# maua-maua-maua/maua

Measured on AMD Instinct MI355X. Metric: frames/sec (whole node), 1024x1024 StyleGAN2 audio-reactive render, higher is better.
Workload: dtype bf16

## Files before the change

maua_amd/csrc/common.h:

```cpp
#pragma once
#include <hip/hip_runtime.h>
#include <stdint.h>
#include <string>

#include "../../include/maua_hip.h"

namespace maua {

typedef __attribute__((ext_vector_type(8))) __bf16 bf16x8;
typedef __attribute__((ext_vector_type(16))) float f32x16;
typedef __attribute__((ext_vector_type(4))) float f32x4;
typedef __attribute__((ext_vector_type(4))) uint32_t u32x4;

typedef uint16_t bf16_t;

__device__ __forceinline__ float bf2f(bf16_t v) { return __uint_as_float(((uint32_t)v) << 16); }
typedef __bf16 hw_bf16x2 __attribute__((ext_vector_type(2)));
typedef float f32x2_t __attribute__((ext_vector_type(2)));
__device__ __forceinline__ uint32_t pack2bf(float lo, float hi) {
  const f32x2_t v = {lo, hi};
  return __builtin_bit_cast(uint32_t, __builtin_convertvector(v, hw_bf16x2));
}
__device__ __forceinline__ bf16_t f2bf(float f) { return (bf16_t)(pack2bf(f, 0.f) & 0xffffu); }

// ... 87 lines not shown

__device__ __forceinline__ void lds_dma_b128(const void* sbase, unsigned voff_bytes, void* lds_wave_base) {
  const unsigned base =
      __builtin_amdgcn_readfirstlane((unsigned)(size_t)(__attribute__((address_space(3))) void*)lds_wave_base);
  asm volatile("s_mov_b32 m0, %2\n\ts_nop 0\n\tglobal_load_lds_dwordx4 %0, %1" ::"v"(voff_bytes), "s"(sbase), "s"(base)
               : "memory");
}

void set_error(const std::string& msg);
int fail(const std::string& msg);
#define MAUA_HIP_CHECK(expr)                                                                  \
  do {                                                                                        \
    hipError_t _e = (expr);                                                                   \
    if (_e != hipSuccess)                                                                     \
      return ::maua::fail(std::string(#expr) + ": " + hipGetErrorString(_e));                 \
  } while (0)
#define MAUA_REQUIRE(cond, msg)                                   \
  do {                                                            \
    if (!(cond)) return ::maua::fail(std::string(msg));           \
  } while (0)

static inline int cdiv(int a, int b) { return (a + b - 1) / b; }

}

struct maua_ctx {
  int device;
  hipStream_t stream;
  void* scratch = nullptr;
  size_t scratch_bytes = 0;
  int dma_conv = 1;
  int gemm_dma = 1;
  int linear_dma = 0;
};

namespace maua {
int scratch_reserve(maua_ctx* ctx, size_t bytes);
}
```

maua_amd/csrc/context.hip:

```cpp
#include "common.h"

namespace maua {
static thread_local std::string g_err;
void set_error(const std::string& msg) { g_err = msg; }
int fail(const std::string& msg) {
  g_err = msg;
  return MAUA_ERR;
}
int scratch_reserve(maua_ctx* ctx, size_t bytes) {
  if (bytes <= ctx->scratch_bytes) return MAUA_OK;
  MAUA_HIP_CHECK(hipStreamSynchronize(ctx->stream));
  if (ctx->scratch) MAUA_HIP_CHECK(hipFree(ctx->scratch));
  ctx->scratch = nullptr;
  ctx->scratch_bytes = 0;
  size_t want = bytes + bytes / 4;
  MAUA_HIP_CHECK(hipMalloc(&ctx->scratch, want));
  ctx->scratch_bytes = want;
  return MAUA_OK;
}
}

namespace {
__global__ void clock_stamp_kernel(unsigned long long* stamp) {
  stamp[0] = __builtin_amdgcn_s_memtime();
// ... 9 lines not shown
int maua_ctx_create(int device, void* stream, maua_ctx** out) {
  MAUA_REQUIRE(out != nullptr, "maua_ctx_create: out is NULL");
  int n = 0;
  MAUA_HIP_CHECK(hipGetDeviceCount(&n));
  MAUA_REQUIRE(device >= 0 && device < n, "maua_ctx_create: no such HIP device (this library has no CPU fallback)");
  MAUA_HIP_CHECK(hipSetDevice(device));
  maua_ctx* c = new maua_ctx();
  c->device = device;
  c->stream = (hipStream_t)stream;
  *out = c;
  return MAUA_OK;
}

int maua_ctx_set_stream(maua_ctx* ctx, void* stream) {
  MAUA_REQUIRE(ctx != nullptr, "maua_ctx_set_stream: ctx is NULL");
  ctx->stream = (hipStream_t)stream;
  return MAUA_OK;
}

int maua_ctx_set_option(maua_ctx* ctx, const char* key, int value) {
  MAUA_REQUIRE(ctx && key, "maua_ctx_set_option: NULL argument");
  if (std::string(key) == "dma_conv") {
    ctx->dma_conv = value;
    return MAUA_OK;
  }
  if (std::string(key) == "linear_dma") {
    ctx->linear_dma = value;
    return MAUA_OK;
  }
  if (std::string(key) == "gemm_dma") {
    ctx->gemm_dma = value;
    return MAUA_OK;
  }
  return maua::fail(std::string("maua_ctx_set_option: unknown option ") + key);
}

int maua_ctx_sync(maua_ctx* ctx) {
  MAUA_REQUIRE(ctx != nullptr, "maua_ctx_sync: ctx is NULL");
  MAUA_HIP_CHECK(hipStreamSynchronize(ctx->stream));
  return MAUA_OK;
}

int maua_ctx_clock_stamp(maua_ctx* ctx, unsigned long long* stamp_dev) {
  MAUA_REQUIRE(ctx && stamp_dev, "maua_ctx_clock_stamp: NULL argument");
  hipLaunchKernelGGL(clock_stamp_kernel, dim3(1), dim3(1), 0, ctx->stream, stamp_dev);
  MAUA_HIP_CHECK(hipGetLastError());
  return MAUA_OK;
}

void maua_ctx_destroy(maua_ctx* ctx) {
  if (!ctx) return;
  if (ctx->scratch) {
    hipStreamSynchronize(ctx->stream);
    hipFree(ctx->scratch);
  }
  delete ctx;
}

}
```

maua_amd/csrc/internal.h:

```cpp
#pragma once
#include "common.h"

namespace maua {

int launch_pack_rgb8(hipStream_t stream, const float* img, uint8_t* out, int B, int H, int W);
template <typename TI, typename TO>
int launch_nchw_to_nhwc(hipStream_t s, const void* x, void* y, int N, int C, int HW, int Cp);
template <typename TI, typename TO>
int launch_nhwc_to_nchw(hipStream_t s, const void* x, void* y, int N, int C, int HW, int Cp);

struct ConvArgs {
  const void* x;
  long x_bstride;
  const void* w;
  const float* s;
  const float* d;
  const float* noise;
  long noise_bstride;
  float noise_strength;
  const float* noise_scale;
  const float* bias;
  void* y;
  int B, H, W, Ci, Co, up;
  int act;
// ... 61 lines not shown
  long noise_bstride;
  float noise_strength;
  const float* noise_scale;
  const float* bias;
  void* y;
  int B, H, W, Ci, Co, up, act;
  float alpha, gain, clamp;
  const float* rgb_wmod;
  const float* rgb_bias;
  const float* rgb_prev;
  float* rgb_out;
  float rgb_clamp;
  float fir[16];
  uint8_t* rgb8_out;
  int rgb_skip_f32;
};
bool hires_supported(int dtype, int Ci, int Co, int up, int H, int W);
int launch_modconv_hires(hipStream_t stream, const HiresArgs& a, int dtype = MAUA_BF16);
bool upwalk_supported(int dtype, int Ci, int Co, int up, int H, int W);
size_t upwalk_weight_elems(int Co, int Ci);
int launch_upwalk(hipStream_t stream, const HiresArgs& a, int dtype = MAUA_BF16);
int launch_prep_upwalk_weights(hipStream_t stream, const float* w, void* wt, int Co, int Ci, int flip, int dtype = MAUA_BF16);
bool upwalk_fused_supported(int dtype, int Ci, int Cm, int H, int W);
int launch_upwalk_fused(hipStream_t stream, const HiresArgs& up, const HiresArgs& c1, int force_segs = 0, int narrow_ok = 1,
                        int dtype = MAUA_BF16);

int launch_prep_weights(hipStream_t stream, int dtype, const float* w, void* wt, float* wsq, int Co, int Ci, int k,
                        int up, int flip, int Cop, int Cip);
int launch_f32_split_inplace(hipStream_t stream, void* w, long n_floats);

int launch_tconv2(hipStream_t stream, int dtype, const ConvArgs& a);
bool tconv_dma_supported(int dtype, int Ci, int Co, int H, int W);
int launch_tconv_dma(hipStream_t stream, const ConvArgs& a, int dtype = MAUA_BF16);
int launch_tconv_edges(hipStream_t stream, const ConvArgs& a, int dtype = MAUA_BF16);
int launch_prep_tconv_weights(hipStream_t stream, int dtype, const float* w, void* wt, int Co, int Ci, int flip);

struct UpfirArgs {
  const void* t;
  void* y;
  const float* d;
  const float* noise;
  long noise_bstride;
  float noise_strength;
  const float* noise_scale;
  const float* bias;
  const float* out_scale;
  int B, H, W, Co;
  int act;
  float alpha, gain, clamp;
};
int launch_upfir_epilogue(hipStream_t stream, int dtype, const UpfirArgs& a);
bool tconv_fir_supported(int dtype, int Ci, int Co, int H, int W);
int launch_tconv_fir(hipStream_t stream, const ConvArgs& a, const UpfirArgs& u, int dtype = MAUA_BF16, int walk = 1, int force_segs = 0);
size_t prepped_weight_elems(int k, int up, int Cop, int Cip);

struct LayerOperands { const void* x; const void* w; const float* s; const float* d; const float* bias; void* y; int B, H, W, Ci, Co, up; };
struct NoiseOperands { const float* noise; long bstride; float strength; const float* scale; };
struct Epilogue { int act; float alpha, gain, clamp; };
template <typename A>
inline void set_noise_args(A& a, const NoiseOperands& n) {
  a.noise = n.noise; a.noise_bstride = n.bstride; a.noise_strength = n.strength; a.noise_scale = n.scale;
}
template <typename A>
inline void set_epilogue_args(A& a, const Epilogue& e) {
  a.act = e.act; a.alpha = e.alpha; a.gain = e.gain; a.clamp = e.clamp;
}
template <typename A>
// ... 60 lines not shown
int launch_resize2d(hipStream_t stream, int dtype, bool nhwc, const ResizeArgs& a);
int launch_skip_add(hipStream_t stream, const float* y, const float* prev, float* out, int B, int H, int W,
                    const float* fir16);
int launch_warp_affine_nhwc(hipStream_t stream, int dtype, const void* x, void* y, const float* minv, int B, int H, int W,
                            int C);

struct StyleLayer {
  const float* affine_w;
  const float* affine_b;
  const float* wsq;
  const float* wrgb;
  float* s;
  float* d;
  float* wmod;
  int w_index;
  int Cin, Co, Cs, Cd;
  float scale;
};
int launch_styles(hipStream_t stream, const StyleLayer* layers_dev, int n_layers, const float* ws, int num_ws,
                  int w_dim, int B, int max_channels, int f16_prenorm = 0);
int launch_f16_prenorm_weights(hipStream_t stream, const float* w, float* out, int Co, int Ci, int kk);
int launch_f16_prenorm_styles(hipStream_t stream, float* s, int B, int Cs, int Cin);

struct RgbArgs {
  const void* x;
  const float* wmod;
  const float* bias;
  const float* prev;
  float* out;
  int B, H, W, C;
  float clamp;
  float fir[16];
};
int launch_torgb(hipStream_t stream, int dtype, const RgbArgs& a);

struct GemmArgs {
  const void* a0; long lda0; int K0;
  const void* a1; long lda1; int K1;
  const void* w;
  const float* bias;
  const void* res;
  long ldr;
  void* c;
  long ldc;
  long M;
  int N;
  int c_f32;
  int prefer_dma;
  int epi;
  void* c2; long ldc2;
  const void* aux; long ldaux;
  int batch;
  long a_bstride, w_bstride, c_bstride;
  int remap_nt;
};
int launch_gemm_nt(hipStream_t stream, int dtype, const GemmArgs& g);
struct GemmRoute { int kernel; int remap_nt; };
GemmRoute gemm_route(int dtype, const GemmArgs& g, int prefer_dma, int force = 0);
int gemm_plan(int dtype, const GemmArgs& g, int prefer_dma, int force, GemmRoute* out);
int launch_gemm_routed(hipStream_t stream, int dtype, const GemmArgs& g, GemmRoute r);
bool gemm_dma_shape_ok(int dtype, const GemmArgs& g);
bool gemm_dma_supported(int dtype, const GemmArgs& g);
bool gemm256_shape_ok(const GemmArgs& g);
bool gemm256_takes(const GemmArgs& g);
int launch_gemm_dma(hipStream_t stream, const GemmArgs& g, int kernel);

struct AttnArgs {
// ... 125 lines not shown
```

maua_amd/csrc/modconv.hip:

```cpp
#include <cstdlib>

#include "common.h"
#include "internal.h"

namespace maua {


template <typename T> struct Mma;
template <> struct Mma<bf16_t> {
  using FW = u32x4;
  using FX = u32x4;
  __device__ static __forceinline__ FW prep_w(const u32x4& v) { return v; }
  __device__ static __forceinline__ FX prep_x(const u32x4& v) { return v; }
  __device__ static __forceinline__ void step(f32x16& acc, const u32x4& a, const u32x4& b) {
    acc = __builtin_amdgcn_mfma_f32_32x32x16_bf16(__builtin_bit_cast(bf16x8, a), __builtin_bit_cast(bf16x8, b), acc, 0,
                                                  0, 0);
  }
  __device__ static __forceinline__ u32x4 scale(const u32x4& v, const float* sv) {
    u32x4 o;
#pragma unroll
    for (int k = 0; k < 4; k++)
      o[k] = pack2bf(bf2f((bf16_t)(v[k] & 0xffff)) * sv[2 * k], bf2f((bf16_t)(v[k] >> 16)) * sv[2 * k + 1]);
    return o;
  }
// ... 872 lines not shown
      if constexpr (sizeof(T) == 2) {
        xv[0] = Fmt16<T>::lo(v.x); xv[1] = Fmt16<T>::hi(v.x);
        xv[2] = Fmt16<T>::lo(v.y); xv[3] = Fmt16<T>::hi(v.y);
        xv[4] = Fmt16<T>::lo(v.z); xv[5] = Fmt16<T>::hi(v.z);
        xv[6] = Fmt16<T>::lo(v.w); xv[7] = Fmt16<T>::hi(v.w);
      } else {
        xv[0] = __uint_as_float(v.x); xv[1] = __uint_as_float(v.y);
        xv[2] = __uint_as_float(v.z); xv[3] = __uint_as_float(v.w);
      }
      float wv[3][EPC];
#pragma unroll
      for (int c = 0; c < 3; c++)
#pragma unroll
        for (int q4 = 0; q4 < EPC / 4; q4++) {
          const f32x4 t = *reinterpret_cast<const f32x4*>(wm + c * a.C + pc * EPC + q4 * 4);
          wv[c][q4 * 4] = t[0]; wv[c][q4 * 4 + 1] = t[1]; wv[c][q4 * 4 + 2] = t[2]; wv[c][q4 * 4 + 3] = t[3];
        }
#pragma unroll
      for (int e = 0; e < EPC; e++) {
        r0 += xv[e] * wv[0][e];
        r1 += xv[e] * wv[1][e];
        r2 += xv[e] * wv[2][e];
      }
    }
    for (int o = LP >> 1; o > 0; o >>= 1) {
      r0 += __shfl_xor(r0, o);
      r1 += __shfl_xor(r1, o);
      r2 += __shfl_xor(r2, o);
    }
    if (sub == 0) torgb_finish(a, b, p, r0, r1, r2);
  }
}

template <int NF>
__global__ __launch_bounds__(256) void torgb_mfma_kernel(RgbArgs a) {
  constexpr int C = NF * 16;
  const int lane = threadIdx.x & 63, r = lane & 31, h = lane >> 5;
  const int b = blockIdx.y;
  u32x4 wf[NF];
  {
    const int c_rgb = r < 3 ? r : (r >= 8 && r < 11 ? r - 8 : -1);
#pragma unroll
    for (int ks = 0; ks < NF; ks++) {
      u32x4 o = u32x4{0u, 0u, 0u, 0u};
      if (c_rgb >= 0) {
        const float* src = a.wmod + ((long)b * 3 + c_rgb) * C + ks * 16 + 8 * h;
        const float4 s0 = *reinterpret_cast<const float4*>(src), s1 = *reinterpret_cast<const float4*>(src + 4);
        const float sv[8] = {s0.x, s0.y, s0.z, s0.w, s1.x, s1.y, s1.z, s1.w};
#pragma unroll
        for (int k = 0; k < 4; k++) {
          float w0 = sv[2 * k], w1 = sv[2 * k + 1];
          const float h0 = bf2f(f2bf(w0)), h1 = bf2f(f2bf(w1));
          if (r >= 8) { w0 -= h0; w1 -= h1; }
          o[k] = pack2bf(w0, w1);
        }
      }
      wf[ks] = o;
    }
  }
  const long HW = (long)a.H * a.W;
  const bf16_t* xb = reinterpret_cast<const bf16_t*>(a.x) + (long)b * HW * C;
  const long n_groups = (HW + 31) / 32;
  for (long gi = (long)blockIdx.x * 4 + (threadIdx.x >> 6); gi < n_groups; gi += (long)gridDim.x * 4) {
    const long p = gi * 32 + r;
    const bf16_t* px = xb + (p < HW ? p : HW - 1) * C + 8 * h;
    u32x4 xv[NF];
#pragma unroll
    for (int ks = 0; ks < NF; ks++) xv[ks] = *reinterpret_cast<const u32x4*>(px + ks * 16);
    f32x16 acc;
#pragma unroll
    for (int e = 0; e < 16; e++) acc[e] = 0.f;
#pragma unroll
    for (int ks = 0; ks < NF; ks++)
      acc = __builtin_amdgcn_mfma_f32_32x32x16_bf16(__builtin_bit_cast(bf16x8, wf[ks]), __builtin_bit_cast(bf16x8, xv[ks]),
                                                    acc, 0, 0, 0);
    if (h == 0 && p < HW) torgb_finish(a, b, p, acc[0] + acc[4], acc[1] + acc[5], acc[2] + acc[6]);
  }
}

int launch_torgb(hipStream_t stream, int dtype, const RgbArgs& a) {
  if (a.B == 0) return MAUA_OK;
  const int epc = dtype == MAUA_F32 ? 4 : 8;
  MAUA_REQUIRE(a.C % epc == 0, "torgb: C must be a multiple of the 16-byte piece");
  if (dtype == MAUA_BF16 && (a.C == 32 || a.C == 64 || a.C == 128 || a.C == 256) && ((uintptr_t)a.wmod % 16) == 0) {
    const long groups = ((long)a.H * a.W + 31) / 32;
    const dim3 grid((unsigned)std::min<long>((groups + 3) / 4, 1024), a.B);
    switch (a.C / 16) {
      case 2: hipLaunchKernelGGL(torgb_mfma_kernel<2>, grid, dim3(256), 0, stream, a); break;
      case 4: hipLaunchKernelGGL(torgb_mfma_kernel<4>, grid, dim3(256), 0, stream, a); break;
      case 8: hipLaunchKernelGGL(torgb_mfma_kernel<8>, grid, dim3(256), 0, stream, a); break;
      default: hipLaunchKernelGGL(torgb_mfma_kernel<16>, grid, dim3(256), 0, stream, a); break;
    }
    MAUA_HIP_CHECK(hipGetLastError());
    return MAUA_OK;
  }
  int pieces = a.C / epc;
  int lp_log2 = 0;
  while ((1 << (lp_log2 + 1)) <= pieces && lp_log2 < 4) lp_log2++;
  long HW = (long)a.H * a.W;
  int ppb = 256 >> lp_log2;
  int gx = (int)std::min<long>((HW + ppb - 1) / ppb, 2048);
  size_t smem = (size_t)3 * a.C * sizeof(float);
  if (dtype == MAUA_BF16)
    hipLaunchKernelGGL(torgb_kernel<bf16_t>, dim3(gx, a.B), dim3(256), smem, stream, a, lp_log2);
  else if (dtype == MAUA_F16)
    hipLaunchKernelGGL(torgb_kernel<f16_t>, dim3(gx, a.B), dim3(256), smem, stream, a, lp_log2);
  else if (dtype == MAUA_F32)
    hipLaunchKernelGGL(torgb_kernel<float>, dim3(gx, a.B), dim3(256), smem, stream, a, lp_log2);
  else
    return fail("torgb: unsupported dtype");
  MAUA_HIP_CHECK(hipGetLastError());
  return MAUA_OK;
}

}
```

maua_amd/csrc/modconv_api.hip:

```cpp
#include <algorithm>
#include <cstring>

#include "common.h"
#include "internal.h"

namespace maua {
namespace {

enum { R_LOWRES = 0, R_GENERIC, R_DMA, R_HIRES, R_UPWALK, R_FUSED, R_WALKDONE, R_TFIR, R_TDMA, R_T2, R_UPFIR };

bool is_tconv(int r) { return r == R_TFIR || r == R_TDMA || r == R_T2; }
bool reads_premod(int r) { return r == R_TFIR || r == R_TDMA || r == R_DMA; }

LayerOperands operands(const maua_modconv_desc* d) {
  return LayerOperands{d->x, nullptr, d->s, d->d, d->bias, d->y, d->B, d->H, d->W, d->Ci, d->Co, d->up};
}
NoiseOperands noise_of(const maua_modconv_desc* d) { return NoiseOperands{d->noise, d->noise_bstride, d->noise_strength, d->noise_scale}; }
Epilogue epilogue_of(const maua_modconv_desc* d) { return Epilogue{d->act, d->alpha, d->gain, d->clamp}; }

template <typename A>
A desc_args(const maua_modconv_desc* d) {
  A a = layer_args(A{}, operands(d), noise_of(d), epilogue_of(d));
  if (d->rgb_out) {
    float fir[16];
// ... 162 lines not shown
  switch (route) {
    case R_LOWRES:
    case R_GENERIC:
    case R_DMA: {
      ConvArgs a = conv_args(d);
      a.x = x; a.x_bstride = x_bstride; a.w = base + o_w;
      if (route == R_DMA) a.s = nullptr;
      return route == R_LOWRES    ? launch_modconv_lowres(st, dtype, a, base + o_xm, (float*)(base + o_ws))
             : route == R_GENERIC ? launch_modconv3x3(st, dtype, a)
                                  : launch_modconv_dma(st, a, dtype);
    }
    case R_HIRES:
    case R_UPWALK:
    case R_FUSED: {
      HiresArgs a = hires_args(d);
      a.w = base + o_w;
      if (route == R_HIRES) return launch_modconv_hires(st, a, dtype);
      if (route == R_UPWALK) return launch_upwalk(st, a, dtype);
      HiresArgs f = hires_args(d1);
      f.x = nullptr; f.y = nullptr; f.w = base + o_w1;
      a.y = nullptr;
      return launch_upwalk_fused(st, a, f, force_segs, narrow_ok, dtype);
    }
    case R_TFIR:
    case R_TDMA:
    case R_T2: {
      void* t = d->t ? d->t : base + o_t;
      ConvArgs a = tconv_args(d);
      a.x = x; a.x_bstride = x_bstride; a.w = base + o_w; a.y = t;
      if (route != R_T2) a.s = (const float*)(base + o_ones);
      UpfirArgs u = upfir_args(d);
      if (route == R_TFIR) return launch_tconv_fir(st, a, u, dtype, force_segs >= 0, force_segs);
      if (route == R_TDMA) {
        if (int rc = launch_tconv_edges(st, a, dtype)) return rc;
        if (int rc = launch_tconv_dma(st, a, dtype)) return rc;
      } else if (int rc = launch_tconv2(st, dtype, a)) {
        return rc;
      }
      u.t = t;
      return launch_upfir_epilogue(st, dtype, u);
    }
    case R_UPFIR: {
      UpfirArgs u = upfir_args(d);
      u.t = d->x;
      return launch_upfir_epilogue(st, dtype, u);
    }
  }
  return MAUA_OK;
}

extern "C" int maua_torgb_ex(maua_ctx* ctx, const void* x, const float* wmod, const float* bias, const float* prev, float* out, int B,
                             int H, int W, int C, float clamp, int dtype) {
  MAUA_REQUIRE(ctx && x && wmod && bias && out, "maua_torgb_ex: NULL argument");
  MAUA_REQUIRE(B >= 0 && H > 0 && W > 0 && C > 0, "maua_torgb_ex: bad shape");
  MAUA_REQUIRE(!prev || (H % 2 == 0 && W % 2 == 0), "maua_torgb_ex: the skip image needs an even grid");
  RgbArgs r{};
  r.x = x; r.wmod = wmod; r.bias = bias; r.prev = prev; r.out = out; r.B = B; r.H = H; r.W = W; r.C = C; r.clamp = clamp;
  upsample_fir16(r.fir);
  return launch_torgb(ctx->stream, dtype, r);
}
```

maua_amd/csrc/modconv_tconv_dma.hip:

```cpp
#include "common.h"
#include "internal.h"

namespace maua {

namespace {

constexpr int PTH = 8, PTW = 32;
constexpr int HW1 = PTW + 1, HPX = (PTH + 1) * HW1;
constexpr int KB = 64;
constexpr int HBUF = HPX * KB;
constexpr int WROWS = 9 * 32;
constexpr int WBUF = WROWS * KB;
constexpr int OFF_H = 2 * WBUF;
constexpr int NW = 4, NT = NW * 64;
constexpr int WJ = (WBUF / 1024 + NW - 1) / NW;
constexpr int HJ = (HPX * 4 + NT - 1) / NT;

__device__ __constant__ const int kSlot[9] = {0, 1, 1, 2, 2, 3, 3, 3, 3};
__device__ __constant__ const int kCls[9] = {0, 0, 1, 0, 2, 0, 1, 2, 3};

__device__ __forceinline__ unsigned lds_off(const void* p) {
  return (unsigned)(size_t)(__attribute__((address_space(3))) const void*)p;
}
__device__ __forceinline__ void dma16_s(const void* sbase, unsigned voff, unsigned lds_dst) {
// ... 188 lines not shown
  f32x16 acc0, acc1;
#pragma unroll
  for (int e = 0; e < 16; e++) { acc0[e] = 0.f; acc1[e] = 0.f; }
  const u32x4 zero = u32x4{0u, 0u, 0u, 0u};
#pragma unroll 4
  for (int k = 0; k < a.Ci; k += 16) {
    const u32x4 A0 = *reinterpret_cast<const u32x4*>(w0 + k), A1 = *reinterpret_cast<const u32x4*>(w1 + k),
                A2 = *reinterpret_cast<const u32x4*>(w2 + k);
    const u32x4 X0 = x0 >= 0 ? *reinterpret_cast<const u32x4*>(xb + x0 + k + 8 * h) : zero;
    const u32x4 X1 = x1 >= 0 ? *reinterpret_cast<const u32x4*>(xb + x1 + k + 8 * h) : zero;
    mma<F>(acc0, A0, X0);
    mma<F>(acc1, A2, X1);
    mma<F>(acc0, A1, X1);
  }
  const int Wt = 2 * a.W + 1, Ht = 2 * a.H + 1;
  uint16_t* yb = reinterpret_cast<uint16_t*>(a.y) + (long)b * Ht * Wt * a.Co + cb * 32 + 4 * h;
  long o0 = -1, o1 = -1;
  if (row_edge) {
    if (e0 <= a.W) o0 = ((long)(2 * a.H) * Wt + 2 * e0) * a.Co;
    if (e0 < a.W) o1 = ((long)(2 * a.H) * Wt + 2 * e0 + 1) * a.Co;
  } else if (e0 < a.H) {
    o0 = ((long)(2 * e0) * Wt + 2 * a.W) * a.Co;
    o1 = ((long)(2 * e0 + 1) * Wt + 2 * a.W) * a.Co;
  }
#pragma unroll
  for (int qd = 0; qd < 4; qd++) {
    if (o0 >= 0)
      *reinterpret_cast<uint2*>(yb + o0 + 8 * qd) = make_uint2(Fmt16<F>::pack2(acc0[qd * 4], acc0[qd * 4 + 1]), Fmt16<F>::pack2(acc0[qd * 4 + 2], acc0[qd * 4 + 3]));
    if (o1 >= 0)
      *reinterpret_cast<uint2*>(yb + o1 + 8 * qd) = make_uint2(Fmt16<F>::pack2(acc1[qd * 4], acc1[qd * 4 + 1]), Fmt16<F>::pack2(acc1[qd * 4 + 2], acc1[qd * 4 + 3]));
  }
}

int tconv_edges_check(const ConvArgs& a, int dtype) {
  MAUA_REQUIRE(dtype == MAUA_BF16 || dtype == MAUA_F16, "tconv_edges: unsupported dtype");
  MAUA_REQUIRE(a.Ci % 16 == 0 && a.Co % 32 == 0, "tconv_edges: Ci % 16, Co % 32");
  MAUA_REQUIRE(a.B <= 65535 && a.Co / 32 <= 65535, "tconv_edges: grid too large");
  return MAUA_OK;
}
int tconv_dma_check(const ConvArgs& a, int dtype) {
  MAUA_REQUIRE(tconv_dma_supported(dtype, a.Ci, a.Co, a.H, a.W), "tconv_dma: unsupported shape");
  const int tiles = (a.H / PTH) * (a.W / PTW), CB = a.Co / 32, cbg = CB < 8 ? CB : 8;
  MAUA_REQUIRE(CB % cbg == 0, "tconv_dma: channel blocks must split into groups of 8");
  const long n_ts = (long)tiles * a.B, grid = ((n_ts + 7) / 8) * 8 * cbg * (CB / cbg);
  MAUA_REQUIRE(grid < (1L << 31), "tconv_dma: grid too large");
  return MAUA_OK;
}

int launch_tconv_edges(hipStream_t stream, const ConvArgs& a, int dtype) {
  if (int rc = tconv_edges_check(a, dtype)) return rc;
  if (a.B == 0) return MAUA_OK;
  const int row_tiles = (a.W + 1 + 31) / 32, col_tiles = (a.H + 31) / 32;
  if (dtype == MAUA_F16)
    hipLaunchKernelGGL(tconv_edges_kernel<f16_t>, dim3(row_tiles + col_tiles, a.B, a.Co / 32), dim3(64), 0, stream, a, row_tiles);
  else
    hipLaunchKernelGGL(tconv_edges_kernel<bf16_t>, dim3(row_tiles + col_tiles, a.B, a.Co / 32), dim3(64), 0, stream, a, row_tiles);
  MAUA_HIP_CHECK(hipGetLastError());
  return MAUA_OK;
}

bool tconv_dma_supported(int dtype, int Ci, int Co, int H, int W) {
  return (dtype == MAUA_BF16 || dtype == MAUA_F16) && Ci % 32 == 0 && Co % 32 == 0 && H % PTH == 0 && W % PTW == 0 &&
         (long)H * W * Ci * 2 < (1L << 32) && 16L * Co * Ci * 2 < (1L << 32);
}

int launch_tconv_dma(hipStream_t stream, const ConvArgs& a, int dtype) {
  if (int rc = tconv_dma_check(a, dtype)) return rc;
  if (a.B == 0) return MAUA_OK;
  const int tiles = (a.H / PTH) * (a.W / PTW), CB = a.Co / 32, cbg = CB < 8 ? CB : 8;
  const long n_ts = (long)tiles * a.B, grid = ((n_ts + 7) / 8) * 8 * cbg * (CB / cbg);
  const size_t smem = std::max<size_t>((size_t)2 * WBUF + 2 * HBUF, (size_t)PTH * PTW * (128 * 2 + 16));
  if (dtype == MAUA_F16) {
    MAUA_HIP_CHECK(hipFuncSetAttribute((const void*)tconv_dma_kernel<f16_t>, hipFuncAttributeMaxDynamicSharedMemorySize, (int)smem));
    hipLaunchKernelGGL(tconv_dma_kernel<f16_t>, dim3((unsigned)grid), dim3(NT), smem, stream, a);
  } else {
    MAUA_HIP_CHECK(hipFuncSetAttribute((const void*)tconv_dma_kernel<bf16_t>, hipFuncAttributeMaxDynamicSharedMemorySize, (int)smem));
    hipLaunchKernelGGL(tconv_dma_kernel<bf16_t>, dim3((unsigned)grid), dim3(NT), smem, stream, a);
  }
  MAUA_HIP_CHECK(hipGetLastError());
  return MAUA_OK;
}

}
```

maua_amd/csrc/synth.hip:

```cpp
#include <cmath>
#include <cstring>
#include <string>
#include <vector>

#include "common.h"
#include "internal.h"

using namespace maua;

namespace {

struct ConvLayer {
  int block, which;
  int Ci, Co, res, up, w_index;
  int ih = 0, iw = 0;
  int oh = 0, ow = 0;
  int fh = 0, fw = 0;
  float* affine_w = nullptr;
  float* affine_b = nullptr;
  float* bias = nullptr;
  float* noise_const = nullptr;
  float noise_strength = 0.f;
  void* wt = nullptr;
  void* wt_t = nullptr;
// ... 10 lines not shown
  float* affine_b = nullptr;
  float* wrgb = nullptr;
  float* bias = nullptr;
  float* s = nullptr;
  float* wmod = nullptr;
};

template <typename T>
int dev_alloc(T** p, size_t n) {
  MAUA_HIP_CHECK(hipMalloc((void**)p, n * sizeof(T)));
  return MAUA_OK;
}

}

struct maua_synth {
  maua_ctx* ctx;
  int res, w_dim, channel_base, channel_max, dtype, nv_compat;
  int nblocks, num_ws;
  size_t esize;
  std::vector<ConvLayer> convs;
  std::vector<RgbLayer> rgbs;
  void* const_x = nullptr;
  int keep_features = 0;
  int lowres = 1;
  int use_hires = 1;
  int upwalk = 2;
  int walk_segs = 0;
  int walk_narrow = 1;
  int fuse_torgb = 1;
  int tconv_up = 1;
  int tconv_fir = 256;
  int tconv_walk = 1;
  const float* nz_scales = nullptr;
  long nz_scale_stride = 0;
  int dma_conv = 1;
  int dual_store = 1;
  int tconv_dma = 1;
  float* ones = nullptr;
  void* xm = nullptr;
  void* tbuf = nullptr;
  void* lowres_xm = nullptr;
  float* lowres_ws = nullptr;
  int rs_layer = -1, rs_mode = 0, rs_th = 0, rs_tw = 0, rs_pl = 0, rs_pr = 0, rs_pt = 0, rs_pb = 0, rs_how = 3;
  float rs_value = 0.f;
  float* rs_noise = nullptr;
  void* const_rs = nullptr;
  float* rgb_tmp[2] = {nullptr, nullptr};
  int out_h = 0, out_w = 0;
  int warp_layer[3] = {-1, -1, -1};
  const float* warp_minv[3] = {nullptr, nullptr, nullptr};
  int profile = 0;
  std::vector<hipEvent_t> ev;
  size_t ev_used = 0;
  std::vector<size_t> ev_fwd_start;
  int bcap = 0;
  void* act[2] = {nullptr, nullptr};
  float* img[2] = {nullptr, nullptr};
  StyleLayer* style_table_dev = nullptr;
  float fir[16];
};

static void prof_mark(maua_synth* n) {
  if (!n->profile || n->ev_used >= (1u << 16)) return;
  if (n->ev_used == n->ev.size()) {
    hipEvent_t e;
// ... 402 lines not shown
  n->warp_layer[slot] = inv_matrices_dev ? layer : -1;
  n->warp_minv[slot] = inv_matrices_dev;
  return MAUA_OK;
}

int maua_synth_layer_size(const maua_synth* n, int layer, int* h, int* w) {
  MAUA_REQUIRE(n && h && w, "maua_synth_layer_size: NULL argument");
  MAUA_REQUIRE(layer >= -1 && layer < (int)n->convs.size(), "maua_synth_layer_size: no such layer");
  if (layer < 0) { *h = n->out_h; *w = n->out_w; }
  else { *h = n->convs[layer].oh; *w = n->convs[layer].ow; }
  return MAUA_OK;
}

int maua_synth_set_option(maua_synth* n, const char* key, int value) {
  MAUA_REQUIRE(n && key, "maua_synth_set_option: NULL argument");
  if (!strcmp(key, "profile")) {
    n->profile = value;
    n->ev_used = 0;
    n->ev_fwd_start.clear();
    return MAUA_OK;
  }
  if (!strcmp(key, "keep_features")) {
    if (n->keep_features != value) {
      MAUA_HIP_CHECK(hipStreamSynchronize(n->ctx->stream));
      free_workspace(n);
      n->keep_features = value;
    }
    return MAUA_OK;
  }
  static const std::pair<const char*, int maua_synth::*> routing[] = {
      {"lowres", &maua_synth::lowres},         {"use_hires", &maua_synth::use_hires}, {"upwalk", &maua_synth::upwalk},
      {"walk_segs", &maua_synth::walk_segs},   {"walk_narrow", &maua_synth::walk_narrow},
      {"fuse_torgb", &maua_synth::fuse_torgb}, {"tconv_up", &maua_synth::tconv_up},   {"tconv_fir", &maua_synth::tconv_fir},
      {"tconv_walk", &maua_synth::tconv_walk},
      {"tconv_dma", &maua_synth::tconv_dma},   {"dma_conv", &maua_synth::dma_conv},   {"dual_store", &maua_synth::dual_store}};
  for (const auto& o : routing)
    if (!strcmp(key, o.first)) {
      n->*o.second = value;
      return MAUA_OK;
    }
  return fail(std::string("maua_synth_set_option: unknown option ") + key);
}

static thread_local hipMemcpyKind g_load_kind = hipMemcpyHostToDevice;

static int upload(float* dst, const float* host, size_t count, size_t expect, const char* name) {
  if (count != expect)
    return fail(std::string("maua_synth_load: ") + name + ": expected " + std::to_string(expect) + " values, got " +
                std::to_string(count));
  MAUA_HIP_CHECK(hipMemcpy(dst, host, count * sizeof(float), g_load_kind));
  return MAUA_OK;
}

int maua_synth_load(maua_synth* n, const char* name, const float* host, size_t count) {
  MAUA_REQUIRE(n && name && host, "maua_synth_load: NULL argument");
  std::string s(name);
  int blk = -1, pos = 0;
  if (sscanf(name, "bs.%d.%n", &blk, &pos) < 1 || blk < 0 || blk >= n->nblocks || pos == 0)
    return fail("maua_synth_load: unknown parameter name: " + s);
  std::string rest = s.substr(pos);
  hipStream_t st = n->ctx->stream;
  auto check_filter = [&]() -> int {
    if (count != 16) return fail("maua_synth_load: " + s + ": only the 4x4 [1,3,3,1] resample filter is supported");
    const float t[4] = {1, 3, 3, 1};
    for (int u = 0; u < 4; u++)
      for (int v = 0; v < 4; v++)
        if (std::fabs(host[u * 4 + v] - t[u] * t[v] / 64.f) > 1e-6f)
// ... 160 lines not shown
          if (s.rgb) fuse_torgb(a);
          if (s.rgb8) pack_u8(a);
          if (s.route != Route::Hires) a.w = c.wt_h;
          if (s.route != Route::FusedWalk) {
            if (int rc = s.route == Route::Hires ? launch_modconv_hires(st, a, n->dtype) : launch_upwalk(st, a, n->dtype)) return rc;
            break;
          }
          HiresArgs f = layer_args(HiresArgs{}, li + 1, nullptr, nullptr);
          fuse_torgb(f);
          if (plan.conv[li + 1].rgb8) pack_u8(f);
          if (int rc = launch_upwalk_fused(st, a, f, n->walk_segs, n->walk_narrow, n->dtype)) return rc;
          break;
        }
        case Route::WalkDone:
          break;
        case Route::TconvFir:
        case Route::TconvDma:
        case Route::Tconv2: {
          ConvArgs a = tconv_args(x, x_bstride, c.wt_t, c.s, n->tbuf, B, c.ih, c.iw, c.Ci, c.Co);
          UpfirArgs u = upfir_args(y, c.d, c.bias, next_s, B, c.ih, c.iw, c.Co, layer_noise(li), lrelu_epilogue());
          if (s.src == Src::PremodPass)
            if (int rc = launch_premod_nhwc(st, x, x_bstride, c.s, n->xm, B, (long)c.ih * c.iw, c.Ci, n->dtype)) return rc;
          if (s.src == Src::PremodPass || s.src == Src::Xm) {
            a.x = n->xm;
            a.x_bstride = (long)c.ih * c.iw * c.Ci;
          }
          if (reads_premod(s.route)) a.s = n->ones;
          if (s.route == Route::TconvFir) {
            if (int rc = launch_tconv_fir(st, a, u, n->dtype, n->tconv_walk, 0)) return rc;
            prof_mark(n);
            break;
          }
          if (s.route == Route::TconvDma) {
            if (int rc = launch_tconv_edges(st, a, n->dtype)) return rc;
            if (int rc = launch_tconv_dma(st, a, n->dtype)) return rc;
          } else if (int rc = launch_tconv2(st, n->dtype, a)) {
            return rc;
          }
          prof_mark(n);
          u.t = n->tbuf;
          if (int rc = launch_upfir_epilogue(st, n->dtype, u)) return rc;
          break;
        }
      }
      prof_mark(n);
      x = y;
      x_bstride = (long)c.oh * c.ow * c.Co;
      cur ^= 1;
      if (hooked) {
        void* dst = n->keep_features ? c.feat : n->act[cur];
        if (int rc = resize_feat(x, x_bstride, B, c.oh, c.ow, c.Co, dst)) return rc;
        x = dst;
        x_bstride = (long)c.fh * c.fw * c.Co;
        cur ^= 1;
      }
      for (int wsl = 0; wsl < 3; wsl++) {
        if (n->warp_layer[wsl] != (int)li + 1 || !n->warp_minv[wsl]) continue;
        void* dst = n->act[cur];
        if (dst == x) dst = n->act[cur ^ 1];
        if (int rc = launch_warp_affine_nhwc(st, n->dtype, x, dst, n->warp_minv[wsl], B, c.fh, c.fw, c.Co)) return rc;
        if (n->keep_features) {
          MAUA_HIP_CHECK(hipMemcpyAsync(c.feat, dst, (size_t)B * c.fh * c.fw * c.Co * n->esize, hipMemcpyDeviceToDevice, st));
        } else {
          x = dst;
          cur = (dst == n->act[0]) ? 1 : 0;
        }
      }
    }
    if (plan.rgb[blk] != RgbRoute::Fused) {
      const bool hook = plan.rgb[blk] == RgbRoute::Hook;
      RgbArgs r{};
      r.x = x; r.wmod = g.wmod; r.bias = g.bias; r.prev = hook ? nullptr : prev_img;
      r.out = hook ? n->rgb_tmp[0] : rgb_out; r.B = B; r.H = g.h; r.W = g.w; r.C = g.C; r.clamp = 256.f;
      memcpy(r.fir, n->fir, sizeof(r.fir));
      if (int rc = launch_torgb(st, n->dtype, r)) return rc;
      if (hook) {
        const ConvLayer& hc = n->convs[n->rs_layer - 1];
        const int nh = hc.oh, nw = hc.ow;
        ResizeArgs inv{};
        inv.x = n->rgb_tmp[0]; inv.x_bstride = 3L * g.h * g.w; inv.y = n->rgb_tmp[1]; inv.B = B; inv.H = g.h; inv.W = g.w;
        inv.C = 3; inv.oh = nh; inv.ow = nw; inv.mode = n->rs_mode; inv.pl = -n->rs_pl; inv.pt = -n->rs_pt;
        inv.how = MAUA_PAD_CONSTANT; inv.value = 0.f; inv.noise = nullptr;
        if (int rc = launch_resize2d(st, MAUA_F32, false, inv)) return rc;
        const float* native = n->rgb_tmp[1];
        if (prev_img) {
          if (int rc = launch_skip_add(st, n->rgb_tmp[1], prev_img, n->rgb_tmp[0], B, nh, nw, n->fir)) return rc;
          native = n->rgb_tmp[0];
        }
        ResizeArgs fwd{};
        fwd.x = native; fwd.x_bstride = 3L * nh * nw; fwd.y = rgb_out; fwd.B = B; fwd.H = nh; fwd.W = nw; fwd.C = 3;
        fwd.oh = g.h; fwd.ow = g.w; fwd.mode = n->rs_mode; fwd.pl = n->rs_pl; fwd.pt = n->rs_pt; fwd.how = n->rs_how;
        fwd.value = n->rs_value; fwd.noise = nullptr;
        if (int rc = launch_resize2d(st, MAUA_F32, false, fwd)) return rc;
      }
    }
    prof_mark(n);
    prev_img = rgb_out;
    img_cur ^= 1;
  }
  if (rgb8_out) {
    if (plan.pack)
      if (int rc = launch_pack_rgb8(st, prev_img, rgb8_out, B, n->out_h, n->out_w)) return rc;
    prof_mark(n);
  }
  return MAUA_OK;
}

int maua_synth_get_plan(maua_synth* n, int want_u8, int* conv_out, int capacity, int* rgb_out, int* pack, int* n_layers) {
// ... 65 lines not shown
```

Baseline: 4563.

## Add LDS-shared tconv edge kernel and register-resident toRGB kernel for C=512

Adds a tconv edge kernel that stages input edge rows and weights through LDS in 64-channel chunks and computes several tiles per block with MFMA across four waves, instead of the per-tile 64-thread kernel. It also adds a toRGB kernel for 512-channel bf16/f16 inputs that keeps the modulated weights in registers, prefetches the next pixel's data, and reduces across 16 lanes with shuffles. Both are on by default through new options. The goal is to cut redundant global loads and raise occupancy on these small kernels, at the cost of more register pressure and new code paths.

```diff
diff --git a/maua_amd/csrc/common.h b/maua_amd/csrc/common.h
--- a/maua_amd/csrc/common.h
+++ b/maua_amd/csrc/common.h
@@ -143,6 +143,8 @@
   int dma_conv = 1;
   int gemm_dma = 1;
   int linear_dma = 0;
+  int edge_share = 1;
+  int torgb_regs = 1;
 };
 
 namespace maua {
diff --git a/maua_amd/csrc/context.hip b/maua_amd/csrc/context.hip
--- a/maua_amd/csrc/context.hip
+++ b/maua_amd/csrc/context.hip
@@ -65,6 +65,14 @@
     ctx->gemm_dma = value;
     return MAUA_OK;
   }
+  if (std::string(key) == "edge_share") {
+    ctx->edge_share = value;
+    return MAUA_OK;
+  }
+  if (std::string(key) == "torgb_regs") {
+    ctx->torgb_regs = value;
+    return MAUA_OK;
+  }
   return maua::fail(std::string("maua_ctx_set_option: unknown option ") + key);
 }
 
diff --git a/maua_amd/csrc/internal.h b/maua_amd/csrc/internal.h
--- a/maua_amd/csrc/internal.h
+++ b/maua_amd/csrc/internal.h
@@ -117,7 +117,7 @@
 int launch_tconv2(hipStream_t stream, int dtype, const ConvArgs& a);
 bool tconv_dma_supported(int dtype, int Ci, int Co, int H, int W);
 int launch_tconv_dma(hipStream_t stream, const ConvArgs& a, int dtype = MAUA_BF16);
-int launch_tconv_edges(hipStream_t stream, const ConvArgs& a, int dtype = MAUA_BF16);
+int launch_tconv_edges(hipStream_t stream, const ConvArgs& a, int dtype = MAUA_BF16, int shared = 1);
 int launch_prep_tconv_weights(hipStream_t stream, int dtype, const float* w, void* wt, int Co, int Ci, int flip);
 
 struct UpfirArgs {
@@ -244,7 +244,7 @@
   float clamp;
   float fir[16];
 };
-int launch_torgb(hipStream_t stream, int dtype, const RgbArgs& a);
+int launch_torgb(hipStream_t stream, int dtype, const RgbArgs& a, int regs = 1);
 
 struct GemmArgs {
   const void* a0; long lda0; int K0;
diff --git a/maua_amd/csrc/modconv.hip b/maua_amd/csrc/modconv.hip
--- a/maua_amd/csrc/modconv.hip
+++ b/maua_amd/csrc/modconv.hip
@@ -928,6 +928,71 @@
   }
 }
 
+template <typename T>
+__global__ __launch_bounds__(256, 3) void torgb_regs_kernel(RgbArgs a) {
+  constexpr int C = 512, LP = 16, NP = C / 8 / LP;
+  __shared__ __attribute__((aligned(16))) float wm[3 * C];
+  const int b = blockIdx.y;
+  for (int i = threadIdx.x; i < 3 * C; i += 256) wm[i] = a.wmod[(long)b * 3 * C + i];
+  __syncthreads();
+  const int sub = threadIdx.x & (LP - 1);
+  float wv[NP][3][8];
+#pragma unroll
+  for (int i = 0; i < NP; i++)
+#pragma unroll
+    for (int c = 0; c < 3; c++)
+#pragma unroll
+      for (int q4 = 0; q4 < 2; q4++) {
+        const f32x4 t = *reinterpret_cast<const f32x4*>(wm + c * C + (sub + LP * i) * 8 + q4 * 4);
+        wv[i][c][q4 * 4] = t[0]; wv[i][c][q4 * 4 + 1] = t[1]; wv[i][c][q4 * 4 + 2] = t[2]; wv[i][c][q4 * 4 + 3] = t[3];
+      }
+  const long HW = (long)a.H * a.W;
+  const T* xb = reinterpret_cast<const T*>(a.x) + (long)b * HW * C;
+  const long step = (long)gridDim.x * 16;
+  long p = (long)blockIdx.x * 16 + (threadIdx.x >> 4);
+  uint4 v[NP], vn[NP];
+  if (p < HW) {
+#pragma unroll
+    for (int i = 0; i < NP; i++) v[i] = *reinterpret_cast<const uint4*>(xb + p * C + (sub + LP * i) * 8);
+  }
+#pragma unroll 1
+  for (; p < HW; p += step) {
+    const T* xn = xb + (p + step < HW ? p + step : p) * C;
+#pragma unroll
+    for (int i = 0; i < NP; i++) vn[i] = *reinterpret_cast<const uint4*>(xn + (sub + LP * i) * 8);
+    __builtin_amdgcn_sched_barrier(0);
+    float r0 = 0.f, r1 = 0.f, r2 = 0.f;
+#pragma unroll
+    for (int i = 0; i < NP; i++) {
+      float xv[8];
+      xv[0] = Fmt16<T>::lo(v[i].x); xv[1] = Fmt16<T>::hi(v[i].x);
+      xv[2] = Fmt16<T>::lo(v[i].y); xv[3] = Fmt16<T>::hi(v[i].y);
+      xv[4] = Fmt16<T>::lo(v[i].z); xv[5] = Fmt16<T>::hi(v[i].z);
+      xv[6] = Fmt16<T>::lo(v[i].w); xv[7] = Fmt16<T>::hi(v[i].w);
+      {
+#pragma clang fp contract(off)
+#pragma unroll
+        for (int e = 0; e < 8; e++) {
+          r0 = __builtin_fmaf(xv[e], wv[i][0][e], r0);
+          r1 = __builtin_fmaf(xv[e], wv[i][1][e], r1);
+          const float p2 = xv[e] * wv[i][2][e];
+          r2 = r2 + p2;
+        }
+      }
+      __builtin_amdgcn_sched_barrier(0);
+    }
+#pragma unroll
+    for (int o = LP >> 1; o > 0; o >>= 1) {
+      r0 += __shfl_xor(r0, o);
+      r1 += __shfl_xor(r1, o);
+      r2 += __shfl_xor(r2, o);
+    }
+    if (sub == 0) torgb_finish(a, b, p, r0, r1, r2);
+#pragma unroll
+    for (int i = 0; i < NP; i++) v[i] = vn[i];
+  }
+}
+
 template <int NF>
 __global__ __launch_bounds__(256) void torgb_mfma_kernel(RgbArgs a) {
   constexpr int C = NF * 16;
@@ -974,10 +1039,20 @@
   }
 }
 
-int launch_torgb(hipStream_t stream, int dtype, const RgbArgs& a) {
+int launch_torgb(hipStream_t stream, int dtype, const RgbArgs& a, int regs) {
   if (a.B == 0) return MAUA_OK;
   const int epc = dtype == MAUA_F32 ? 4 : 8;
   MAUA_REQUIRE(a.C % epc == 0, "torgb: C must be a multiple of the 16-byte piece");
+  if (regs && a.C == 512 && (dtype == MAUA_BF16 || dtype == MAUA_F16)) {
+    const long groups = ((long)a.H * a.W + 15) / 16;
+    const dim3 grid((unsigned)std::min<long>(groups, std::max(1, cdiv(768, a.B))), a.B);
+    if (dtype == MAUA_BF16)
+      hipLaunchKernelGGL(torgb_regs_kernel<bf16_t>, grid, dim3(256), 0, stream, a);
+    else
+      hipLaunchKernelGGL(torgb_regs_kernel<f16_t>, grid, dim3(256), 0, stream, a);
+    MAUA_HIP_CHECK(hipGetLastError());
+    return MAUA_OK;
+  }
   if (dtype == MAUA_BF16 && (a.C == 32 || a.C == 64 || a.C == 128 || a.C == 256) && ((uintptr_t)a.wmod % 16) == 0) {
     const long groups = ((long)a.H * a.W + 31) / 32;
     const dim3 grid((unsigned)std::min<long>((groups + 3) / 4, 1024), a.B);
diff --git a/maua_amd/csrc/modconv_api.hip b/maua_amd/csrc/modconv_api.hip
--- a/maua_amd/csrc/modconv_api.hip
+++ b/maua_amd/csrc/modconv_api.hip
@@ -218,7 +218,7 @@
       UpfirArgs u = upfir_args(d);
       if (route == R_TFIR) return launch_tconv_fir(st, a, u, dtype, force_segs >= 0, force_segs);
       if (route == R_TDMA) {
-        if (int rc = launch_tconv_edges(st, a, dtype)) return rc;
+        if (int rc = launch_tconv_edges(st, a, dtype, ctx->edge_share)) return rc;
         if (int rc = launch_tconv_dma(st, a, dtype)) return rc;
       } else if (int rc = launch_tconv2(st, dtype, a)) {
         return rc;
@@ -243,5 +243,5 @@
   RgbArgs r{};
   r.x = x; r.wmod = wmod; r.bias = bias; r.prev = prev; r.out = out; r.B = B; r.H = H; r.W = W; r.C = C; r.clamp = clamp;
   upsample_fir16(r.fir);
-  return launch_torgb(ctx->stream, dtype, r);
-}
+  return launch_torgb(ctx->stream, dtype, r, ctx->torgb_regs);
+}
diff --git a/maua_amd/csrc/modconv_tconv_dma.hip b/maua_amd/csrc/modconv_tconv_dma.hip
--- a/maua_amd/csrc/modconv_tconv_dma.hip
+++ b/maua_amd/csrc/modconv_tconv_dma.hip
@@ -244,6 +244,146 @@
   }
 }
 
+constexpr int EMT = 4, ENT = 2;
+constexpr int EKC = 64;
+constexpr int ERS = EKC * 2 + 16;
+constexpr int EXR = EMT * 33, EWR = ENT * 3 * 32;
+constexpr int EXJ = (EXR * 8 + NT - 1) / NT;
+constexpr int EWJ = EWR * 8 / NT;
+static_assert(EWR * 8 % NT == 0 && NW == (EMT / 2) * ENT, "tconv_edges_shared: four waves = 2 tile pairs x 2 channel blocks");
+
+template <typename F>
+__global__ __launch_bounds__(NT, 3) void tconv_edges_shared_kernel(ConvArgs a, int g_row, int g_col) {
+  __shared__ __attribute__((aligned(16))) char sm[(EXR + EWR) * ERS];
+  char* smx = sm;
+  char* smw = sm + EXR * ERS;
+  const int tid = threadIdx.x, lane = tid & 63, r = lane & 31, h = lane >> 5;
+  const int wave = __builtin_amdgcn_readfirstlane(tid >> 6);
+  const int CB = a.Co >> 5;
+  int g = blockIdx.x, kind = 0;
+  if (g >= g_row + g_col) { kind = 2; g -= g_row + g_col; }
+  else if (g >= g_row) { kind = 1; g -= g_row; }
+  const int tiles = kind == 0 ? (a.W + 31) >> 5 : (a.H + 31) >> 5;
+  const int n_ct = kind == 2 ? (a.B + 31) >> 5 : a.B * tiles;
+  const int ct0 = g * EMT, cb0 = blockIdx.y * ENT;
+  const uint16_t* xp = reinterpret_cast<const uint16_t*>(a.x);
+  const uint16_t* wp = reinterpret_cast<const uint16_t*>(a.w);
+
+  const int q = tid & 7, row0 = tid >> 3;
+  long xo[EXJ];
+#pragma unroll
+  for (int j = 0; j < EXJ; j++) {
+    const int row = row0 + 32 * j, m = row / 33, rr = row - m * 33, ct = ct0 + m;
+    long o = -1;
+    if (row < EXR && ct < n_ct) {
+      if (kind == 2) {
+        const int b = ct * 32 + rr;
+        if (rr < 32 && b < a.B) o = (long)b * a.x_bstride + ((long)(a.H - 1) * a.W + (a.W - 1)) * a.Ci;
+      } else {
+        const int b = ct / tiles, e = (ct - b * tiles) * 32 + rr - 1;
+        if (kind == 0 && e >= 0 && e < a.W) o = (long)b * a.x_bstride + ((long)(a.H - 1) * a.W + e) * a.Ci;
+        if (kind == 1 && e >= 0 && e < a.H) o = (long)b * a.x_bstride + ((long)e * a.W + (a.W - 1)) * a.Ci;
+      }
+    }
+    xo[j] = o < 0 ? -1 : o + q * 8;
+  }
+  const int s1 = kind == 1 ? 2 : 1;
+  const long wt = (long)row0 * a.Ci + q * 8;
+  long wblk[EWJ];
+#pragma unroll
+  for (int j = 0; j < EWJ; j++) {
+    const int cbl = j / 3, blk = j - cbl * 3, cb = cb0 + cbl;
+    const int slot = blk == 0 ? 0 : s1, cls = blk == 2 ? s1 : 0;
+    wblk[j] = cb < CB ? (((long)slot * CB + cb) * 4 + cls) * 32 * a.Ci : -1;
+  }
+
+  const u32x4 zero = u32x4{0u, 0u, 0u, 0u};
+  u32x4 sx[EXJ], sw[EWJ];
+#define TE_LOAD(C_)                                                                                       \
+  {                                                                                                       \
+    const int k0_ = (C_) * EKC;                                                                           \
+    const bool in_ = k0_ + q * 8 < a.Ci;                                                                  \
+    _Pragma("unroll") for (int j = 0; j < EXJ; j++)                                                      \
+      sx[j] = in_ && xo[j] >= 0 ? *reinterpret_cast<const u32x4*>(xp + xo[j] + k0_) : zero;               \
+    _Pragma("unroll") for (int j = 0; j < EWJ; j++)                                                      \
+      sw[j] = in_ && wblk[j] >= 0 ? *reinterpret_cast<const u32x4*>(wp + wblk[j] + k0_ + wt) : zero;      \
+  }
+
+  const int ctp = wave & 1, cbl = wave >> 1;
+  const bool active = cb0 + cbl < CB;
+  f32x16 acc0[2], acc1[2];
+#pragma unroll
+  for (int t = 0; t < 2; t++)
+#pragma unroll
+    for (int e = 0; e < 16; e++) { acc0[t][e] = 0.f; acc1[t][e] = 0.f; }
+
+  const int n_chunks = (a.Ci + EKC - 1) / EKC;
+  TE_LOAD(0)
+  for (int c = 0; c < n_chunks; c++) {
+    if (c > 0) __syncthreads();
+#pragma unroll
+    for (int j = 0; j < EXJ; j++)
+      if (row0 + 32 * j < EXR) *reinterpret_cast<u32x4*>(smx + (row0 + 32 * j) * ERS + q * 16) = sx[j];
+#pragma unroll
+    for (int j = 0; j < EWJ; j++) *reinterpret_cast<u32x4*>(smw + (row0 + 32 * j) * ERS + q * 16) = sw[j];
+    __syncthreads();
+    if (c + 1 < n_chunks) TE_LOAD(c + 1)
+    const int nks = min(EKC, a.Ci - c * EKC) >> 4;
+    if (active) {
+#pragma unroll
+      for (int ks = 0; ks < EKC / 16; ks++) {
+        if (ks < nks) {
+          const int bo = ks * 32 + h * 16;
+          const char* wb = smw + (cbl * 3 * 32 + r) * ERS + bo;
+          const u32x4 A0 = *reinterpret_cast<const u32x4*>(wb), A1 = *reinterpret_cast<const u32x4*>(wb + 32 * ERS),
+                      A2 = *reinterpret_cast<const u32x4*>(wb + 64 * ERS);
+#pragma unroll
+          for (int t = 0; t < 2; t++) {
+            const char* xr = smx + ((2 * ctp + t) * 33 + r) * ERS + bo;
+            const u32x4 X0 = *reinterpret_cast<const u32x4*>(xr);
+            const u32x4 X1 = kind == 2 ? zero : *reinterpret_cast<const u32x4*>(xr + ERS);
+            mma<F>(acc0[t], A0, X0);
+            mma<F>(acc1[t], A2, X1);
+            mma<F>(acc0[t], A1, X1);
+          }
+        }
+      }
+    }
+  }
+#undef TE_LOAD
+  if (!active) return;
+  const int Wt = 2 * a.W + 1, Ht = 2 * a.H + 1;
+  uint16_t* yp = reinterpret_cast<uint16_t*>(a.y) + (cb0 + cbl) * 32 + 4 * h;
+#pragma unroll
+  for (int t = 0; t < 2; t++) {
+    const int ct = ct0 + 2 * ctp + t;
+    long o0 = -1, o1 = -1;
+    if (ct < n_ct) {
+      if (kind == 2) {
+        const int b = ct * 32 + r;
+        if (b < a.B) o0 = ((long)b * Ht * Wt + (long)(2 * a.H) * Wt + 2 * a.W) * a.Co;
+      } else {
+        const int b = ct / tiles, e0 = (ct - b * tiles) * 32 + r;
+        if (kind == 0 && e0 < a.W) {
+          o0 = ((long)b * Ht * Wt + (long)(2 * a.H) * Wt + 2 * e0) * a.Co;
+          o1 = o0 + a.Co;
+        }
+        if (kind == 1 && e0 < a.H) {
+          o0 = ((long)b * Ht * Wt + (long)(2 * e0) * Wt + 2 * a.W) * a.Co;
+          o1 = o0 + (long)Wt * a.Co;
+        }
+      }
+    }
+#pragma unroll
+    for (int qd = 0; qd < 4; qd++) {
+      if (o0 >= 0)
+        *reinterpret_cast<uint2*>(yp + o0 + 8 * qd) = make_uint2(Fmt16<F>::pack2(acc0[t][qd * 4], acc0[t][qd * 4 + 1]), Fmt16<F>::pack2(acc0[t][qd * 4 + 2], acc0[t][qd * 4 + 3]));
+      if (o1 >= 0)
+        *reinterpret_cast<uint2*>(yp + o1 + 8 * qd) = make_uint2(Fmt16<F>::pack2(acc1[t][qd * 4], acc1[t][qd * 4 + 1]), Fmt16<F>::pack2(acc1[t][qd * 4 + 2], acc1[t][qd * 4 + 3]));
+    }
+  }
+}
+
 int tconv_edges_check(const ConvArgs& a, int dtype) {
   MAUA_REQUIRE(dtype == MAUA_BF16 || dtype == MAUA_F16, "tconv_edges: unsupported dtype");
   MAUA_REQUIRE(a.Ci % 16 == 0 && a.Co % 32 == 0, "tconv_edges: Ci % 16, Co % 32");
@@ -259,9 +399,20 @@
   return MAUA_OK;
 }
 
-int launch_tconv_edges(hipStream_t stream, const ConvArgs& a, int dtype) {
+int launch_tconv_edges(hipStream_t stream, const ConvArgs& a, int dtype, int shared) {
   if (int rc = tconv_edges_check(a, dtype)) return rc;
   if (a.B == 0) return MAUA_OK;
+  if (shared) {
+    const long g_row = ((long)a.B * cdiv(a.W, 32) + EMT - 1) / EMT, g_col = ((long)a.B * cdiv(a.H, 32) + EMT - 1) / EMT;
+    const long g_cor = (cdiv(a.B, 32) + EMT - 1) / EMT;
+    const dim3 grid((unsigned)(g_row + g_col + g_cor), cdiv(a.Co / 32, ENT));
+    if (dtype == MAUA_F16)
+      hipLaunchKernelGGL(tconv_edges_shared_kernel<f16_t>, grid, dim3(NT), 0, stream, a, (int)g_row, (int)g_col);
+    else
+      hipLaunchKernelGGL(tconv_edges_shared_kernel<bf16_t>, grid, dim3(NT), 0, stream, a, (int)g_row, (int)g_col);
+    MAUA_HIP_CHECK(hipGetLastError());
+    return MAUA_OK;
+  }
   const int row_tiles = (a.W + 1 + 31) / 32, col_tiles = (a.H + 31) / 32;
   if (dtype == MAUA_F16)
     hipLaunchKernelGGL(tconv_edges_kernel<f16_t>, dim3(row_tiles + col_tiles, a.B, a.Co / 32), dim3(64), 0, stream, a, row_tiles);
diff --git a/maua_amd/csrc/synth.hip b/maua_amd/csrc/synth.hip
--- a/maua_amd/csrc/synth.hip
+++ b/maua_amd/csrc/synth.hip
@@ -66,6 +66,8 @@
   int tconv_up = 1;
   int tconv_fir = 256;
   int tconv_walk = 1;
+  int edge_share = 1;
+  int torgb_regs = 1;
   const float* nz_scales = nullptr;
   long nz_scale_stride = 0;
   int dma_conv = 1;
@@ -534,7 +536,7 @@
       {"lowres", &maua_synth::lowres},         {"use_hires", &maua_synth::use_hires}, {"upwalk", &maua_synth::upwalk},
       {"walk_segs", &maua_synth::walk_segs},   {"walk_narrow", &maua_synth::walk_narrow},
       {"fuse_torgb", &maua_synth::fuse_torgb}, {"tconv_up", &maua_synth::tconv_up},   {"tconv_fir", &maua_synth::tconv_fir},
-      {"tconv_walk", &maua_synth::tconv_walk},
+      {"tconv_walk", &maua_synth::tconv_walk}, {"edge_share", &maua_synth::edge_share}, {"torgb_regs", &maua_synth::torgb_regs},
       {"tconv_dma", &maua_synth::tconv_dma},   {"dma_conv", &maua_synth::dma_conv},   {"dual_store", &maua_synth::dual_store}};
   for (const auto& o : routing)
     if (!strcmp(key, o.first)) {
@@ -761,7 +763,7 @@
             break;
           }
           if (s.route == Route::TconvDma) {
-            if (int rc = launch_tconv_edges(st, a, n->dtype)) return rc;
+            if (int rc = launch_tconv_edges(st, a, n->dtype, n->edge_share)) return rc;
             if (int rc = launch_tconv_dma(st, a, n->dtype)) return rc;
           } else if (int rc = launch_tconv2(st, n->dtype, a)) {
             return rc;
@@ -802,7 +804,7 @@
       r.x = x; r.wmod = g.wmod; r.bias = g.bias; r.prev = hook ? nullptr : prev_img;
       r.out = hook ? n->rgb_tmp[0] : rgb_out; r.B = B; r.H = g.h; r.W = g.w; r.C = g.C; r.clamp = 256.f;
       memcpy(r.fir, n->fir, sizeof(r.fir));
-      if (int rc = launch_torgb(st, n->dtype, r)) return rc;
+      if (int rc = launch_torgb(st, n->dtype, r, n->torgb_regs)) return rc;
       if (hook) {
         const ConvLayer& hc = n->convs[n->rs_layer - 1];
         const int nh = hc.oh, nw = hc.ow;
```

New measurement: 4602, median of 6. No clear change (+0.8%).
